# Luoyadan/CRB-active-3Ddet

Hardware: AMD Instinct MI355X
Metric: frames/s SECOND fwd+bwd, KITTI 20k-pt clouds (higher is better)
Workload: dtype f32

## Files before the change

crb-active-3ddet_amd/crbhip/bnrelu.py:

```python
import torch

from ._lib import lib, check, ptr, cur_stream, require_cuda


FUSE_RUNNING = __import__('os').environ.get('CRB_BN_FUSE_RUNNING', '1') == '1'
TICKETS = __import__('os').environ.get('CRB_BN_TICKETS', '1') == '1'
_ticket_areas = {}


def _scratch(dev, wsb):
    ws = torch.empty((wsb,), dtype=torch.uint8, device=dev)
    if not TICKETS:
        return ws, None
    key = (dev.index, torch.cuda.current_stream(dev).cuda_stream)
    t = _ticket_areas.get(key)
    if t is None:
        t = _ticket_areas[key] = torch.zeros((lib.crb_bn_ticket_ints(),), dtype=torch.int32, device=dev)
    return ws, t


def _bn_check(rc, what):
    if rc != 0:
        _ticket_areas.clear()
    check(rc, what)
# ... 260 lines not shown
            zptr = ctypes.c_void_p(out.data_ptr() + 4 * col)
            _bn_check(lib.crb_bn_relu_forward(ptr(x), n, C, ptr(g), ptr(b), float(eps), int(relu), zptr, total, ptr(mean),
                                          ptr(var), ptr(invstd), ptr(rm), ptr(rv), None, float(mom), ptr(ws), wsb, ptr(tk),
                                          cur_stream(dev)), 'crb_bn_relu_forward')
            _touch(rm, rv)
            saved += [x, mean, invstd, g, b]
            col += C
        ctx.save_for_backward(*saved)
        ctx.relu, ctx.widths = int(relu), widths
        return out

    @staticmethod
    def backward(ctx, dz):
        import ctypes
        dz = dz.contiguous().float()
        n, total = dz.shape
        saved = ctx.saved_tensors
        grads, col = [None], 0
        for i, C in enumerate(ctx.widths):
            x, mean, invstd, g, b = saved[5 * i:5 * i + 5]
            dev = x.device
            dx = torch.empty_like(x)
            dgamma = torch.empty((C,), dtype=torch.float32, device=dev)
            dbeta = torch.empty_like(dgamma)
            wsb = lib.crb_bn_workspace_bytes(n, C)
            ws, tk = _scratch(dev, wsb)
            dzp = ctypes.c_void_p(dz.data_ptr() + 4 * col)
            _bn_check(lib.crb_bn_relu_backward(ptr(x), dzp, total, n, C, ptr(mean), ptr(invstd), ptr(g), ptr(b), ctx.relu,
                                           ptr(dx), ptr(dgamma), ptr(dbeta), ptr(ws), wsb, ptr(tk), cur_stream(dev)),
                  'crb_bn_relu_backward')
            grads += [dx, dgamma, dbeta, None, None, None, None]
            col += C
        return tuple(grads)


def bn_relu_concat(xs, bns, relu=True):
    if _GROUPS is not None and _GROUPS.G > 1:
        off = _GROUPS.offsets(xs[0])
        if not torch.is_grad_enabled():
            total = sum(x.shape[1] for x in xs)
            out = torch.empty((xs[0].shape[0], total), dtype=torch.float32, device=xs[0].device)
            col = 0
            for x, bn in zip(xs, bns):
                _frames_forward(x, off, bn, relu, out, col)
                col += x.shape[1]
            return out
        with frame_groups(1):
            return torch.cat([bn_relu_concat([x[a:b] for x in xs], bns, relu) for a, b in zip(off[:-1], off[1:])], 0)
    args = []
    for x, bn in zip(xs, bns):
        with torch.no_grad():
            bn.num_batches_tracked += 1
        args += [x, bn.weight, bn.bias, bn.eps, bn.running_mean, bn.running_var, float(bn.momentum)]
    return _BNReLUConcatTrain.apply(relu, *args)


class _BNReLUMaxConcatTrain(torch.autograd.Function):

    @staticmethod
    def forward(ctx, *args):
        import ctypes
        k = len(args) // 8
        xs = [args[8 * i].contiguous() for i in range(k)]
        nss = [int(args[8 * i + 1]) for i in range(k)]
        dev = xs[0].device
        M = xs[0].shape[0] // nss[0]
        widths = [x.shape[1] for x in xs]
        total = sum(widths)
        out = torch.empty((M, total), dtype=torch.float32, device=dev)
        saved, col = [], 0
        for i, x in enumerate(xs):
            gamma, beta, eps, rm, rv, mom = args[8 * i + 2:8 * i + 8]
            C, ns = widths[i], nss[i]
            assert x.shape[0] == M * ns
            mean = torch.empty((C,), dtype=torch.float32, device=dev)
            var, invstd = torch.empty_like(mean), torch.empty_like(mean)
            arg = torch.empty((M, C), dtype=torch.int32, device=dev)
            wsb = lib.crb_bn_workspace_bytes(M * ns, C)
            ws, tk = _scratch(dev, wsb)
            g, b = gamma.contiguous().float(), beta.contiguous().float()
            zptr = ctypes.c_void_p(out.data_ptr() + 4 * col)
            _bn_check(lib.crb_bn_relu_max_forward(ptr(x), M, ns, C, ptr(g), ptr(b), float(eps), zptr, total, ptr(arg),
                                              ptr(mean), ptr(var), ptr(invstd), ptr(rm), ptr(rv), None, float(mom), ptr(ws), wsb,
                                              ptr(tk), cur_stream(dev)), 'crb_bn_relu_max_forward')
            _touch(rm, rv)
            saved += [x, mean, invstd, g, b, arg]
            col += C
        ctx.save_for_backward(*saved)
        ctx.widths, ctx.nss = widths, nss
        return out

    @staticmethod
    def backward(ctx, gz):
        import ctypes
        gz = gz.contiguous().float()
        M, total = gz.shape
        saved = ctx.saved_tensors
        grads, col = [], 0
        for i, (C, ns) in enumerate(zip(ctx.widths, ctx.nss)):
            x, mean, invstd, g, b, arg = saved[6 * i:6 * i + 6]
            dev = x.device
            dx = torch.empty_like(x)
            dgamma = torch.empty((C,), dtype=torch.float32, device=dev)
            dbeta = torch.empty_like(dgamma)
            wsb = lib.crb_bn_workspace_bytes(M * ns, C)
            ws, tk = _scratch(dev, wsb)
            gp = ctypes.c_void_p(gz.data_ptr() + 4 * col)
# ... 46 lines not shown
```

crb-active-3ddet_amd/csrc/bn_relu.hip:

```cpp
#include "crb_common.h"
#include "../../include/crb_hip.h"

typedef float f4 __attribute__((ext_vector_type(4)));

namespace {

static inline int bn_rows_per_block(int64_t n) {
  int64_t r = (n + 1023) / 1024;
  r = r < 128 ? 128 : r;
  return (int)r;
}

CRB_KNOB g_bn_order = 2;

constexpr int BN_GROUPS = 32;
struct BnFinal {
  int* tickets;
  double* group;
  float* o0;
  float* o1;
  float* o2;
  float* running_mean;
  float* running_var;
  long long* num_batches_tracked;
  float momentum, eps;
  int64_t n;
  int bwd;
};

__device__ __forceinline__ void st_agent(float* p, float v) {
  __hip_atomic_store(p, v, __ATOMIC_RELAXED, __HIP_MEMORY_SCOPE_AGENT);
}
__device__ __forceinline__ void st_agent4(float* p, f4 v) {
  st_agent(p, v[0]);
  st_agent(p + 1, v[1]);
  st_agent(p + 2, v[2]);
  st_agent(p + 3, v[3]);
}

__device__ __forceinline__ void bn_ticket_finalize(const float* partial, int nblk, int C, int blk, const BnFinal& f) {
  __shared__ int s_role;
  asm volatile("s_waitcnt vmcnt(0)" ::: "memory");
  __syncthreads();
  const int ngroups = nblk < BN_GROUPS ? nblk : BN_GROUPS;
  const int grp = blk % BN_GROUPS;
  const int members = (nblk - grp + BN_GROUPS - 1) / BN_GROUPS;
  if (threadIdx.x == 0)
    s_role = __hip_atomic_fetch_add(&f.tickets[1 + grp], 1, __ATOMIC_RELAXED, __HIP_MEMORY_SCOPE_AGENT) == members - 1 ? 1 : 0;
  __syncthreads();
  if (!s_role) return;
  const int C2 = 2 * C;
  for (int i = threadIdx.x; i < C2; i += 256) {
    double a = 0.0;
    int k = grp;
    for (; k + 7 * BN_GROUPS < nblk; k += 8 * BN_GROUPS) {
      float v[8];
// ... 387 lines not shown
                                                              const float* __restrict__ gamma, const float* __restrict__ beta,
                                                              float* __restrict__ z, int C, int relu, int64_t ld_z,
                                                              BnFrames fr) {
  const int f = blockIdx.y;
  const int64_t rows = fr.off[f + 1] - fr.off[f];
  const int64_t t = (int64_t)blockIdx.x * 256 + threadIdx.x;
  if (t * 4 >= rows * C) return;
  const int c = (int)((t * 4) % C);
  const int64_t row = fr.off[f] + (t * 4) / C;
  const float* st = stats + (int64_t)f * 4 * C;
  const f4 v = *reinterpret_cast<const f4*>(x + row * C + c);
  const f4 mu = *reinterpret_cast<const f4*>(st + c), is = *reinterpret_cast<const f4*>(st + 2 * C + c);
  const f4 ga = *reinterpret_cast<const f4*>(gamma + c), be = *reinterpret_cast<const f4*>(beta + c);
  f4 o = ga * ((v - mu) * is) + be;
  if (relu) {
#pragma unroll
    for (int k = 0; k < 4; ++k) o[k] = o[k] > 0.f ? o[k] : 0.f;
  }
  *reinterpret_cast<f4*>(z + row * ld_z + c) = o;
}

__global__ __launch_bounds__(256) void bn_relu_max_frames_kernel(const float* __restrict__ x, const float* __restrict__ stats,
                                                                 const float* __restrict__ gamma, const float* __restrict__ beta,
                                                                 int64_t groups, int64_t groups_per_frame, int ns, int C,
                                                                 float* __restrict__ zmax, int64_t ld_out,
                                                                 int* __restrict__ arg) {
  const int c4n = C >> 2;
  const int tc = threadIdx.x % c4n, tr = threadIdx.x / c4n;
  const int glanes = 256 / c4n;
  if (tr >= glanes) return;
  const int64_t m = (int64_t)blockIdx.x * glanes + tr;
  if (m >= groups) return;
  const int c = tc * 4;
  const float* st = stats + (m / groups_per_frame) * 4 * C;
  const f4 mu = *reinterpret_cast<const f4*>(st + c), is = *reinterpret_cast<const f4*>(st + 2 * C + c);
  const f4 ga = *reinterpret_cast<const f4*>(gamma + c), be = *reinterpret_cast<const f4*>(beta + c);
  const float* src = x + m * ns * C + c;
  f4 best = (f4){-1.f, -1.f, -1.f, -1.f};
  int bi[4] = {0, 0, 0, 0};
  for (int s = 0; s < ns; ++s) {
    const f4 v = *reinterpret_cast<const f4*>(src + (int64_t)s * C);
    f4 o = ga * ((v - mu) * is) + be;
#pragma unroll
    for (int k = 0; k < 4; ++k) {
      o[k] = o[k] > 0.f ? o[k] : 0.f;
      if (o[k] > best[k]) { best[k] = o[k]; bi[k] = s; }
    }
  }
  *reinterpret_cast<f4*>(zmax + m * ld_out + c) = best;
  int* a = arg + m * C + c;
  a[0] = bi[0]; a[1] = bi[1]; a[2] = bi[2]; a[3] = bi[3];
}

}

static inline int bn_blocks(int64_t n) { return crb_cdiv(n, bn_rows_per_block(n)); }

static inline int64_t bn_partial_bytes(int64_t n, int C) { return crb_align_up((int64_t)bn_blocks(n) * 2 * C * 4, 256); }
extern "C" int64_t crb_bn_workspace_bytes(int64_t n, int C) {
  return bn_partial_bytes(n, C) + (int64_t)BN_GROUPS * 2 * C * 8 + 256;
}
extern "C" int crb_bn_ticket_ints(void) { return 1 + BN_GROUPS; }

static inline BnFinal bn_final(int32_t* tickets, void* workspace, int64_t n, int C, int bwd, float* o0, float* o1, float* o2,
                               float* running_mean, float* running_var, float momentum, float eps,
                               int64_t* num_batches_tracked = nullptr) {
  BnFinal f;
  f.tickets = tickets;
  f.group = reinterpret_cast<double*>(static_cast<char*>(workspace) + bn_partial_bytes(n, C));
  f.o0 = o0;
  f.o1 = o1;
  f.o2 = o2;
  f.running_mean = running_mean;
  f.running_var = running_var;
  f.num_batches_tracked = reinterpret_cast<long long*>(num_batches_tracked);
  f.momentum = momentum;
  f.eps = eps;
  f.n = n;
  f.bwd = bwd;
  return f;
}

extern "C" int crb_bn_relu_forward(const float* x, int64_t n, int C, const float* gamma, const float* beta, float eps,
                                   int relu, float* z, int64_t z_row_stride, float* mean, float* var, float* invstd,
                                   float* running_mean, float* running_var, int64_t* num_batches_tracked, float momentum,
                                   void* workspace, int64_t workspace_bytes, int32_t* tickets, void* stream) {
  const int64_t ld_z = z_row_stride > 0 ? z_row_stride : C;
  if (ld_z < C || (ld_z & 3)) return CRB_ERR_ARG;
  if (n <= 0 || C <= 0 || (C & 3) || C > 1024 || (256 % (C >> 2) && (C >> 2) < 256)) return CRB_ERR_ARG;
  if (workspace_bytes < crb_bn_workspace_bytes(n, C) - 256 || !workspace) return CRB_ERR_WORKSPACE;
  hipStream_t st = (hipStream_t)stream;
  const int nblk = bn_blocks(n);
  float* partial = (float*)workspace;
  hipLaunchKernelGGL(bn_partial_kernel<false>, dim3(nblk), dim3(256), 2 * 256 * 16, st, x, nullptr, nullptr, nullptr,
                     nullptr, nullptr, n, C, relu, bn_rows_per_block(n), (int64_t)C, partial, g_bn_order & 1,
                     bn_final(tickets, workspace, n, C, 0, mean, var, invstd, running_mean, running_var, momentum, eps,
                              num_batches_tracked));
  if (!tickets)
    hipLaunchKernelGGL(bn_finalize_kernel, dim3(crb_cdiv(C, 8)), dim3(256), 0, st, partial, nblk, C, n, eps, 0, mean, var,
                       invstd, running_mean, running_var, momentum, reinterpret_cast<long long*>(num_batches_tracked));
  const int64_t total4 = n * C / 4;
  if (z)
    hipLaunchKernelGGL(bn_apply_kernel, dim3(crb_cdiv(total4, 256)), dim3(256), 0, st, x, mean, invstd, gamma, beta, z,
                       total4, C, relu, ld_z, (g_bn_order >> 1) & 1);
  CRB_CHECK_LAUNCH();
  return CRB_OK;
// ... 25 lines not shown
  if (workspace_bytes < crb_bn_workspace_bytes(n, C) - 256 || !workspace) return CRB_ERR_WORKSPACE;
  hipStream_t st = (hipStream_t)stream;
  const int nblk = (int)(n_slabs < bn_blocks(n) ? n_slabs : bn_blocks(n));
  float* partial = (float*)workspace;
  hipLaunchKernelGGL(bn_slab_partial_kernel, dim3(nblk), dim3(256), 0, st, slab_sums, n_slabs, C, partial,
                     bn_final(tickets, workspace, n, C, 0, mean, var, invstd, running_mean, running_var, momentum, eps,
                              num_batches_tracked));
  if (!tickets)
    hipLaunchKernelGGL(bn_finalize_kernel, dim3(crb_cdiv(C, 8)), dim3(256), 0, st, partial, nblk, C, n, eps, 0, mean, var,
                       invstd, running_mean, running_var, momentum, reinterpret_cast<long long*>(num_batches_tracked));
  const int64_t total4 = n * C / 4;
  if (z)
    hipLaunchKernelGGL(bn_apply_kernel, dim3(crb_cdiv(total4, 256)), dim3(256), 0, st, x, mean, invstd, gamma, beta, z,
                       total4, C, relu, ld_z, (g_bn_order >> 1) & 1);
  CRB_CHECK_LAUNCH();
  return CRB_OK;
}

extern "C" int crb_bn_relu_apply(const float* x, int64_t n, int C, const float* mean, const float* invstd,
                                 const float* gamma, const float* beta, int relu, float* z, int64_t z_row_stride,
                                 void* stream) {
  if (n < 0 || C <= 0 || (C & 3)) return CRB_ERR_ARG;
  const int64_t ld_z = z_row_stride > 0 ? z_row_stride : C;
  if (ld_z < C || (ld_z & 3)) return CRB_ERR_ARG;
  if (n == 0) return CRB_OK;
  const int64_t total4 = n * C / 4;
  hipLaunchKernelGGL(bn_apply_kernel, dim3(crb_cdiv(total4, 256)), dim3(256), 0, (hipStream_t)stream, x, mean, invstd,
                     gamma, beta, z, total4, C, relu, ld_z, 0);
  CRB_CHECK_LAUNCH();
  return CRB_OK;
}

extern "C" int crb_bn_relu_backward(const float* x, const float* dz, int64_t dz_row_stride, int64_t n, int C, const float* mean,
                                    const float* invstd, const float* gamma, const float* beta, int relu, float* dx,
                                    float* dgamma, float* dbeta, void* workspace, int64_t workspace_bytes, int32_t* tickets,
                                    void* stream) {
  if (n <= 0 || C <= 0 || (C & 3) || C > 1024 || (256 % (C >> 2) && (C >> 2) < 256)) return CRB_ERR_ARG;
  if (workspace_bytes < crb_bn_workspace_bytes(n, C) - 256 || !workspace) return CRB_ERR_WORKSPACE;
  const int64_t ld_dz = dz_row_stride > 0 ? dz_row_stride : C;
  if (ld_dz < C || (ld_dz & 3)) return CRB_ERR_ARG;
  hipStream_t st = (hipStream_t)stream;
  const int nblk = bn_blocks(n);
  float* partial = (float*)workspace;
  hipLaunchKernelGGL(bn_partial_kernel<true>, dim3(nblk), dim3(256), 2 * 256 * 16, st, x, dz, mean, invstd, gamma, beta, n,
                     C, relu, bn_rows_per_block(n), ld_dz, partial, g_bn_order & 1,
                     bn_final(tickets, workspace, n, C, 1, dbeta, dgamma, nullptr, nullptr, nullptr, 0.f, 0.f));
  if (!tickets)
    hipLaunchKernelGGL(bn_finalize_kernel, dim3(crb_cdiv(C, 8)), dim3(256), 0, st, partial, nblk, C, n, 0.f, 1, dbeta, dgamma,
                       (float*)nullptr, (float*)nullptr, (float*)nullptr, 0.f);
  const int64_t total4 = n * C / 4;
  if (dx)
    hipLaunchKernelGGL(bn_bwd_apply_kernel, dim3(crb_cdiv(total4, 256)), dim3(256), 0, st, x, dz, mean, invstd, gamma, beta,
                       dbeta, dgamma, dx, total4, C, 1.0f / (float)n, relu, ld_dz, (g_bn_order >> 1) & 1);
  CRB_CHECK_LAUNCH();
  return CRB_OK;
}

#ifdef CRB_MEASURE
extern "C" int crb_bn_relu_backward_partials(const float* x, const float* dz, int64_t dz_row_stride, int64_t n, int C,
                                             const float* slab_sums, int64_t n_slabs, const float* mean, const float* invstd,
                                             const float* gamma, const float* beta, int relu, float* dx, float* dgamma, float* dbeta,
                                             void* workspace, int64_t workspace_bytes, int32_t* tickets, void* stream) {
  if (n <= 0 || C <= 0 || (C & 3) || C > 1024 || (256 % (C >> 2) && (C >> 2) < 256) || !slab_sums || n_slabs <= 0) return CRB_ERR_ARG;
  if (workspace_bytes < crb_bn_workspace_bytes(n, C) - 256 || !workspace) return CRB_ERR_WORKSPACE;
  const int64_t ld_dz = dz_row_stride > 0 ? dz_row_stride : C;
  if (ld_dz < C || (ld_dz & 3)) return CRB_ERR_ARG;
  hipStream_t st = (hipStream_t)stream;
  const int nblk = (int)(n_slabs < bn_blocks(n) ? n_slabs : bn_blocks(n));
  float* partial = (float*)workspace;
  hipLaunchKernelGGL(bn_slab_partial_kernel, dim3(nblk), dim3(256), 0, st, slab_sums, n_slabs, C, partial,
                     bn_final(tickets, workspace, n, C, 1, dbeta, dgamma, nullptr, nullptr, nullptr, 0.f, 0.f));
  if (!tickets)
    hipLaunchKernelGGL(bn_finalize_kernel, dim3(crb_cdiv(C, 8)), dim3(256), 0, st, partial, nblk, C, n, 0.f, 1, dbeta, dgamma,
                       (float*)nullptr, (float*)nullptr, (float*)nullptr, 0.f);
  const int64_t total4 = n * C / 4;
  if (dx)
    hipLaunchKernelGGL(bn_bwd_apply_kernel, dim3(crb_cdiv(total4, 256)), dim3(256), 0, st, x, dz, mean, invstd, gamma, beta,
                       dbeta, dgamma, dx, total4, C, 1.0f / (float)n, relu, ld_dz, (g_bn_order >> 1) & 1);
  CRB_CHECK_LAUNCH();
  return CRB_OK;
}
#endif

extern "C" int crb_bn_relu_max_forward(const float* x, int64_t groups, int ns, int C, const float* gamma, const float* beta,
                                       float eps, float* zmax, int64_t out_row_stride, int32_t* arg, float* mean, float* var,
                                       float* invstd, float* running_mean, float* running_var,
                                       int64_t* num_batches_tracked, float momentum, void* workspace,
                                       int64_t workspace_bytes, int32_t* tickets, void* stream) {
  const int64_t n = groups * ns;
  const int64_t ld = out_row_stride > 0 ? out_row_stride : C;
  if (ld < C || (ld & 3) || ns <= 0) return CRB_ERR_ARG;
  if (n <= 0 || C <= 0 || (C & 3) || C > 1024 || (256 % (C >> 2) && (C >> 2) < 256)) return CRB_ERR_ARG;
  if (workspace_bytes < crb_bn_workspace_bytes(n, C) - 256 || !workspace) return CRB_ERR_WORKSPACE;
  hipStream_t st = (hipStream_t)stream;
  const int nblk = bn_blocks(n);
  float* partial = (float*)workspace;
  hipLaunchKernelGGL(bn_partial_kernel<false>, dim3(nblk), dim3(256), 2 * 256 * 16, st, x, nullptr, nullptr, nullptr,
                     nullptr, nullptr, n, C, 1, bn_rows_per_block(n), (int64_t)C, partial, 0,
                     bn_final(tickets, workspace, n, C, 0, mean, var, invstd, running_mean, running_var, momentum, eps,
                              num_batches_tracked));
  if (!tickets)
    hipLaunchKernelGGL(bn_finalize_kernel, dim3(crb_cdiv(C, 8)), dim3(256), 0, st, partial, nblk, C, n, eps, 0, mean, var,
                       invstd, running_mean, running_var, momentum, reinterpret_cast<long long*>(num_batches_tracked));
  const int glanes = 256 / (C >> 2) > 0 ? 256 / (C >> 2) : 1;
  hipLaunchKernelGGL(bn_relu_max_kernel, dim3(crb_cdiv(groups, glanes)), dim3(256), 0, st, x, mean, invstd, gamma, beta,
                     groups, ns, C, zmax, ld, arg);
// ... 172 lines not shown
```

crb-active-3ddet_amd/pcdet/models/backbones_2d/base_bev_backbone.py:

```python
import numpy as np
import torch
import torch.nn as nn

from crbhip import bnrelu

from ...utils.fold_utils import fold_conv_bn
from ...utils.linear_rows import LinearRows, rows_view, rows_to_nchw


ROWS_TRAIN = True
ROWS_GEMM = True
WINOGRAD = __import__('os').environ.get('CRB_WINOGRAD', '1') != '0'


def _wino_fold(w, shift):
    from crbhip import winograd
    return winograd.weights_forward2(w), shift.contiguous()


def _wino_ok(conv, x, pad=None):
    if not WINOGRAD or not isinstance(conv, nn.Conv2d) or not x.is_cuda or x.dtype != torch.float32:
        return False
    from crbhip import winograd
    p = tuple(conv.padding) if pad is None else tuple(pad)
# ... 189 lines not shown
    def forward(self, data_dict):
        spatial_features = data_dict['spatial_features']
        ups = []
        x = spatial_features
        if not self.training and not torch.is_grad_enabled():
            cat_ok = x.is_cuda and x.is_contiguous(memory_format=torch.channels_last) and self._can_fuse_concat_eval(x)
            pre = []
            for i, blk in enumerate(self.blocks):
                x = self._run_folded(blk, x)
                if cat_ok:
                    pre.append(self._up(self.deblocks[i][0], x))
                else:
                    ups.append(self._run_folded(self.deblocks[i], x) if len(self.deblocks) > 0 else x)
            if cat_ok and all(p.is_contiguous(memory_format=torch.channels_last) and p.shape[2:] == pre[0].shape[2:]
                              for p in pre):
                n, _, h, w_ = pre[0].shape
                cat = torch.empty((n * h * w_, sum(p.shape[1] for p in pre)), dtype=torch.float32, device=x.device)
                col = 0
                for d, p in zip(self.deblocks, pre):
                    bnrelu.bn_apply_into(p.permute(0, 2, 3, 1).reshape(n * h * w_, p.shape[1]), d[1], True, cat, col)
                    col += p.shape[1]
                ups = [cat.view(n, h, w_, cat.shape[1]).permute(0, 3, 1, 2)]
            elif cat_ok:
                ups = [self._run_folded(nn.Sequential(*list(d)[1:]), p) for d, p in zip(self.deblocks, pre)]
            x = torch.cat(ups, dim=1) if len(ups) > 1 else ups[0]
            if len(self.deblocks) > len(self.blocks):
                x = self._run_folded(self.deblocks[-1], x)
            data_dict['spatial_features_2d'] = x
            return data_dict
        run = self._run_rows_train if (ROWS_TRAIN and x.is_cuda and x.is_contiguous(memory_format=torch.channels_last)) \
            else (lambda seq, t: seq(t))
        if run == self._run_rows_train and torch.is_grad_enabled():
            from crbhip import winograd
            if winograd.PREPARE:
                winograd.prepare_weights2([m.weight for blk in self.blocks for m in blk
                                           if isinstance(m, nn.Conv2d) and m.kernel_size == (3, 3) and m.stride == (1, 1)
                                           and m.weight.is_cuda])
        fuse_cat = ROWS_TRAIN and x.is_cuda and self._can_fuse_concat(x)
        pre = []
        for i, blk in enumerate(self.blocks):
            x = run(blk, x)
            stride = int(spatial_features.shape[2] / x.shape[2])
            data_dict['spatial_features_%dx' % stride] = x
            if fuse_cat:
                pre.append(self._up(self.deblocks[i][0], x))
            else:
                ups.append(run(self.deblocks[i], x) if len(self.deblocks) > 0 else x)
        if fuse_cat and all(p.is_contiguous(memory_format=torch.channels_last) and p.shape[2:] == pre[0].shape[2:]
                            for p in pre):
            n, _, h, w_ = pre[0].shape
            rows = [p.permute(0, 2, 3, 1).reshape(n * h * w_, p.shape[1]) for p in pre]
            cat = bnrelu.bn_relu_concat(rows, [d[1] for d in self.deblocks[:len(pre)]], relu=True)
            ups = [cat.view(n, h, w_, cat.shape[1]).permute(0, 3, 1, 2)]
        elif fuse_cat:
            ups = [d[2](d[1](p)) for d, p in zip(self.deblocks, pre)]
        x = torch.cat(ups, dim=1) if len(ups) > 1 else ups[0]
        if len(self.deblocks) > len(self.blocks):
            x = self.deblocks[-1](x)
        data_dict['spatial_features_2d'] = x
        if x.is_cuda:
            from crbhip import winograd
            winograd.forget_prepared_forward()
        return data_dict
```

crb-active-3ddet_amd/pcdet/models/dense_heads/anchor_head_single.py:

```python
import numpy as np
import torch
import torch.nn as nn

from ...utils.linear_rows import LinearRows, rows_view
from .anchor_head_template import AnchorHeadTemplate


FUSED_HEAD_CONVS = True
ROWS_GEMM = True


class AnchorHeadSingle(AnchorHeadTemplate):
    def __init__(self, model_cfg, input_channels, num_class, class_names, grid_size, point_cloud_range,
                 predict_boxes_when_training=True, **kwargs):
        super().__init__(model_cfg=model_cfg, num_class=num_class, class_names=class_names, grid_size=grid_size,
                         point_cloud_range=point_cloud_range, predict_boxes_when_training=predict_boxes_when_training)
        self.num_anchors_per_location = sum(self.num_anchors_per_location)
        n = self.num_anchors_per_location
        self.conv_cls = nn.Conv2d(input_channels, n * self.num_class, kernel_size=1)
        self.conv_box = nn.Conv2d(input_channels, n * self.box_coder.code_size, kernel_size=1)
        if self.model_cfg.get('USE_DIRECTION_CLASSIFIER', None) is not None:
            self.conv_dir_cls = nn.Conv2d(input_channels, n * self.model_cfg.NUM_DIR_BINS, kernel_size=1)
        else:
            self.conv_dir_cls = None
        self.lazy_box_decode = False
        self.init_weights()

    def init_weights(self):
        pi = 0.01
        nn.init.constant_(self.conv_cls.bias, -np.log((1 - pi) / pi))
        nn.init.normal_(self.conv_box.weight, mean=0, std=0.001)

    def forward(self, data_dict):
        feats = data_dict['spatial_features_2d']
        if FUSED_HEAD_CONVS:
            heads = [self.conv_cls, self.conv_box] + ([self.conv_dir_cls] if self.conv_dir_cls is not None else [])
            w = torch.cat([h.weight for h in heads], 0)
            b = torch.cat([h.bias for h in heads], 0)
            rows = rows_view(feats) if (ROWS_GEMM and feats.is_cuda) else None
            if rows is not None:
                n, _, h, w_ = feats.shape
                y = LinearRows.apply(rows, w.flatten(1), b).view(n, h, w_, w.shape[0])
            else:
                y = torch.nn.functional.conv2d(feats, w, b).permute(0, 2, 3, 1)
            outs = torch.split(y, [h.out_channels for h in heads], dim=3)
            cls_preds, box_preds = outs[0].contiguous(), outs[1].contiguous()
            dir_cls_preds = outs[2].contiguous() if self.conv_dir_cls is not None else None
        else:
            cls_preds = self.conv_cls(feats).permute(0, 2, 3, 1).contiguous()
            box_preds = self.conv_box(feats).permute(0, 2, 3, 1).contiguous()
            dir_cls_preds = None
            if self.conv_dir_cls is not None:
                dir_cls_preds = self.conv_dir_cls(feats).permute(0, 2, 3, 1).contiguous()
        self.forward_ret_dict['cls_preds'] = cls_preds
        self.forward_ret_dict['box_preds'] = box_preds
        self.forward_ret_dict['dir_cls_preds'] = dir_cls_preds
        if self.training:
            self.forward_ret_dict.update(self.assign_targets(gt_boxes=data_dict['gt_boxes']))
        if not self.training or self.predict_boxes_when_training:
            B = data_dict['batch_size']
            data_dict['rpn_preds'] = cls_preds
            data_dict['cls_preds_normalized'] = False
            if self.lazy_box_decode:
                data_dict['batch_cls_preds'] = cls_preds.view(B, -1, self.num_class).float()
                data_dict['batch_box_decoder'] = lambda idx: self.generate_predicted_boxes(
                    batch_size=B, cls_preds=cls_preds, box_preds=box_preds, dir_cls_preds=dir_cls_preds, anchor_idx=idx)[1]
                data_dict.pop('batch_box_preds', None)
            else:
                batch_cls_preds, batch_box_preds = self.generate_predicted_boxes(
                    batch_size=B, cls_preds=cls_preds, box_preds=box_preds, dir_cls_preds=dir_cls_preds)
                data_dict['batch_cls_preds'] = batch_cls_preds
                data_dict['batch_box_preds'] = batch_box_preds
        return data_dict
```

include/crb_hip.h:

```cpp
#ifndef CRB_HIP_H
#define CRB_HIP_H
#include <stdint.h>

#ifdef __cplusplus
extern "C" {
#endif

#define CRB_OK 0
#define CRB_ERR_ARG (-1)
#define CRB_ERR_WORKSPACE (-2)
#define CRB_ERR_LAUNCH (-3)
#define CRB_ERR_UNSUPPORTED (-4)

int crb_abi_version(void);

int64_t crb_voxelize_workspace_bytes(int64_t n_points, int B, int max_voxels, int max_points);
int crb_voxelize(const float* points, int64_t n_points, int num_features,
                 const int32_t* frame_offsets, int B,
                 const float* range_min_xyz, const float* voxel_size_xyz, const int32_t* grid_xyz,
                 int max_voxels, int max_points,
                 float* voxels, int32_t* coords, int32_t* num_points, float* mean_features,
                 int32_t* num_voxels_out,
                 void* workspace, int64_t workspace_bytes, void* stream);

// ... 223 lines not shown
int64_t crb_pair_sort_workspace_bytes(int64_t M, int nsample);
int crb_pair_sort_by_source(int B, int64_t M, int nsample, const int32_t* xyz_batch_cnt, const int32_t* new_xyz_batch_cnt,
                            const int32_t* idx, const uint8_t* empty_mask, int64_t n_src, int32_t* sorted_pair,
                            int32_t* sorted_row, void* workspace, int64_t workspace_bytes, void* stream);
int crb_sorted_key_counts(const void* key, int key_is_float, int64_t stride, int64_t n, int B, int32_t* counts, void* stream);
int crb_voxel_centers(const int32_t* coords_zyx, int64_t row_stride, int64_t n, const float* scaled_voxel_size, const float* range_min,
                      float* out, void* stream);
int crb_farthest_point_sample(int B, int n, int m, const float* xyz, float* temp, int32_t* out_idx, void* stream);
int crb_three_nn_stack(int B, int64_t N, const float* unknown, const int32_t* unknown_batch_cnt,
                       const float* known, const int32_t* known_batch_cnt, float* dist2, int32_t* idx,
                       void* stream);
int crb_three_interpolate_stack(int64_t N, int C, const float* features, const int32_t* idx,
                                const float* weight, float* out, void* stream);
int crb_three_interpolate_grad_stack(int64_t N, int C, const float* grad_out, const int32_t* idx,
                                     const float* weight, float* grad_features, void* stream);

int crb_points_in_boxes(int B, int T, int M, const float* boxes, const float* pts, int32_t* box_idx_of_points,
                        void* stream);
int64_t crb_gt_point_stats_workspace_bytes(int B, int G, int C);
int crb_gt_point_stats(int B, int G, int C, int64_t N, int stride, const float* pts, const int32_t* frame_offsets,
                       const float* gt_boxes, float* stats, void* workspace, int64_t workspace_bytes, void* stream);
int crb_roiaware_pool3d_forward(int N, int P, int C, int max_pts_each_voxel, int out_x, int out_y, int out_z,
                                const float* rois, const float* pts, const float* pts_feature,
                                int32_t* argmax, int32_t* pts_idx_of_voxels, float* pooled_features,
                                int pool_method, void* stream);
int crb_roiaware_pool3d_backward(int N, int C, int max_pts_each_voxel, int out_x, int out_y, int out_z,
                                 const int32_t* pts_idx_of_voxels, const int32_t* argmax,
                                 const float* grad_out, float* grad_in, int pool_method, void* stream);

int64_t crb_density_greedy_workspace_bytes(int n_candidates, int num_class);
int crb_density_greedy(const float* densities, const int32_t* labels, int n_candidates, int dmax,
                       int num_class, const double* xaxis, const double* prior, double bandwidth,
                       int select_nums, int32_t* order, double* best_scores, void* workspace,
                       int64_t workspace_bytes, void* stream);

int64_t crb_bn_workspace_bytes(int64_t n, int C);
int crb_bn_ticket_ints(void);
int crb_bn_relu_forward(const float* x, int64_t n, int C, const float* gamma, const float* beta, float eps,
                        int relu, float* z, int64_t z_row_stride, float* mean, float* var, float* invstd,
                        float* running_mean, float* running_var, int64_t* num_batches_tracked, float momentum,
                        void* workspace, int64_t workspace_bytes, int32_t* tickets, void* stream);
int crb_bn_relu_forward_partials(const float* x, int64_t n, int C, const float* slab_sums, int64_t n_slabs, const float* gamma,
                                 const float* beta, float eps, int relu, float* z, int64_t z_row_stride, float* mean, float* var,
                                 float* invstd, float* running_mean, float* running_var, int64_t* num_batches_tracked,
                                 float momentum, void* workspace, int64_t workspace_bytes, int32_t* tickets, void* stream);
int crb_bn_affine_table(const float* mean, const float* invstd, const float* gamma, const float* beta, int C, float* out_c2,
                        void* stream);
int crb_bn_relu_apply(const float* x, int64_t n, int C, const float* mean, const float* invstd,
                      const float* gamma, const float* beta, int relu, float* z, int64_t z_row_stride, void* stream);
int crb_bn_relu_backward(const float* x, const float* dz, int64_t dz_row_stride, int64_t n, int C, const float* mean,
                         const float* invstd, const float* gamma, const float* beta, int relu, float* dx,
                         float* dgamma, float* dbeta, void* workspace, int64_t workspace_bytes, int32_t* tickets,
                         void* stream);
int crb_bn_relu_max_forward(const float* x, int64_t groups, int ns, int C, const float* gamma, const float* beta, float eps,
                            float* zmax, int64_t out_row_stride, int32_t* arg, float* mean, float* var, float* invstd,
                            float* running_mean, float* running_var, int64_t* num_batches_tracked, float momentum,
                            void* workspace, int64_t workspace_bytes, int32_t* tickets, void* stream);
int crb_bn_relu_max_backward(const float* x, const float* gz, int64_t gz_row_stride, const int32_t* arg, int64_t groups,
                             int ns, int C, const float* mean, const float* invstd, const float* gamma, const float* beta,
                             float* dx, float* dgamma, float* dbeta, void* workspace, int64_t workspace_bytes,
                             int32_t* tickets, void* stream);
int crb_bn_relu_max_backward_sums(const float* x_sel, const float* gz, int64_t gz_row_stride, int64_t groups, int C,
                                  const float* mean, const float* invstd, const float* gamma, const float* beta, float* dgamma,
                                  float* dbeta, void* workspace, int64_t workspace_bytes, int32_t* tickets, void* stream);
int64_t crb_bn_frames_workspace_bytes(int n_frames, int64_t max_rows_per_frame, int C);
int crb_bn_relu_forward_frames(const float* x, int n_frames, const int64_t* frame_row_offsets, int C, const float* gamma,
                               const float* beta, float eps, int relu, float* z, int64_t z_row_stride,
                               float* running_mean, float* running_var, float momentum, void* workspace,
                               int64_t workspace_bytes, void* stream);
int crb_bn_relu_max_forward_frames(const float* x, int n_frames, int64_t groups_per_frame, int ns, int C,
                                   const float* gamma, const float* beta, float eps, float* zmax, int64_t out_row_stride,
                                   int32_t* arg, float* running_mean, float* running_var, float momentum, void* workspace,
                                   int64_t workspace_bytes, void* stream);

int64_t crb_assign_targets_workspace_bytes(int B, int A, int G);
int crb_assign_targets(const float* anchors, const int32_t* anchor_cls, int A, const float* gt_boxes,
                       const uint8_t* gt_valid, int B, int G, const float* matched_thr,
                       const float* unmatched_thr, int32_t* labels, float* reg_targets, float* reg_weights,
                       void* workspace, int64_t workspace_bytes, void* stream);

typedef struct CrbRpnLossCfg {
  float alpha, gamma;
  float beta;
  float dir_offset;
  float code_weights[7];
  float cls_weight, loc_weight, dir_weight;
  int32_t num_class, num_dir_bins;
} CrbRpnLossCfg;
int64_t crb_rpn_loss_workspace_bytes(int B, int A);
int crb_rpn_loss_forward(const float* cls_preds, const float* box_preds, const float* dir_preds, const int32_t* labels,
                         const float* reg_targets, const float* anchors, int B, int A, const CrbRpnLossCfg* cfg,
                         float* loss, float* npos, void* workspace, int64_t workspace_bytes, void* stream);
int crb_rpn_loss_backward(const float* cls_preds, const float* box_preds, const float* dir_preds, const int32_t* labels,
                          const float* reg_targets, const float* anchors, int B, int A, const CrbRpnLossCfg* cfg,
                          const float* npos, const float* grad_loss, float* d_cls, float* d_box, float* d_dir, void* stream);

int crb_decode_selected_anchors(const float* box_preds, const float* dir_preds, const float* anchors, const int64_t* anchor_idx, int B,
                                int64_t A, int k, int num_dir_bins, float dir_offset, float dir_limit_offset, float* out, void* stream);
int crb_proposal_finish(const int32_t* keep, const int64_t* top_idx, const float* top_boxes, const float* scores, const int64_t* labels,
                        const float* cls_preds, int B, int64_t A, int k, int post, int box_row_stride, int num_class, float* rois,
                        float* roi_scores, int64_t* roi_labels, float* full_cls_scores, void* stream);

int crb_point_labels(const int32_t* inner, const int32_t* outer, const float* gt_boxes, int B, int64_t M, int G, int gt_row_stride,
                     int num_class, int64_t* labels, void* stream);
int crb_point_focal_loss(const float* preds, const int64_t* labels, int64_t n, int num_class, float alpha, float gamma,
                         float loss_weight, float* loss, float* d_preds, void* stream);
// ... 217 lines not shown
```

Measured before the change: 480.2.

## Fuse detection-head GEMM backward into BN-ReLU-concat backward via low-rank MFMA kernels

Adds a fused autograd path for the BEV concat feeding the 1x1 head conv. The head's input gradient (dy·W) is recomputed on the fly per 16-row tile with MFMA inside the BN-ReLU backward partial and apply kernels, so the wide concat gradient never has to be materialised. The aim is to avoid writing and reading back the full n×C_total activation gradient. In exchange the small GEMM is computed twice (once in the partial pass, once in the apply pass), and the path depends on tensor data_ptr matching, supported channel widths, and K ≤ 72.

```diff
diff --git a/crb-active-3ddet_amd/crbhip/bnrelu.py b/crb-active-3ddet_amd/crbhip/bnrelu.py
--- a/crb-active-3ddet_amd/crbhip/bnrelu.py
+++ b/crb-active-3ddet_amd/crbhip/bnrelu.py
@@ -336,7 +336,81 @@
         with torch.no_grad():
             bn.num_batches_tracked += 1
         args += [x, bn.weight, bn.bias, bn.eps, bn.running_mean, bn.running_var, float(bn.momentum)]
-    return _BNReLUConcatTrain.apply(relu, *args)
+    out = _BNReLUConcatTrain.apply(relu, *args)
+    if CONCAT_HEAD and out.grad_fn is not None:
+        out._crb_concat_head = ConcatHandle(out, xs, bns, out.grad_fn.saved_tensors, relu)
+    return out
+
+
+CONCAT_HEAD = __import__('os').environ.get('CRB_CONCAT_HEAD', '1') == '1'
+
+
+class ConcatHandle(object):
+
+    def __init__(self, cat, xs, bns, saved, relu):
+        self.key = (cat.data_ptr(), tuple(cat.shape))
+        self.xs, self.bns, self.saved, self.relu = list(xs), list(bns), tuple(saved), int(relu)
+        self.widths = [int(x.shape[1]) for x in xs]
+
+    def matches(self, rows):
+        return rows.data_ptr() == self.key[0] and tuple(rows.shape) == self.key[1] and rows.is_contiguous()
+
+
+def concat_head_supported(handle, rows, K):
+    return (CONCAT_HEAD and handle is not None and torch.is_grad_enabled() and handle.matches(rows) and
+            all(lib.crb_bn_relu_backward_lowrank_supported(C, int(K)) == 1 for C in handle.widths))
+
+
+class _ConcatHead(torch.autograd.Function):
+
+    @staticmethod
+    def forward(ctx, cat, w, b, handle, *leaves):
+        ctx.save_for_backward(cat, w, *handle.saved)
+        ctx.relu, ctx.widths = handle.relu, handle.widths
+        return torch.addmm(b, cat, w.t())
+
+    @staticmethod
+    def backward(ctx, dy):
+        import ctypes
+        from pcdet.utils.linear_rows import tall_t_matmul
+        saved = ctx.saved_tensors
+        cat, w = saved[0], saved[1]
+        dy = dy.contiguous().float()
+        n, K = dy.shape
+        total = w.shape[1]
+        w = w.contiguous()
+        dw = tall_t_matmul(dy, cat) if ctx.needs_input_grad[1] else None
+        db = dy.sum(0) if ctx.needs_input_grad[2] else None
+        grads, col = [None, dw, db, None], 0
+        for i, C in enumerate(ctx.widths):
+            x, mean, invstd, g, be = saved[2 + 5 * i:7 + 5 * i]
+            need = ctx.needs_input_grad[4 + 3 * i:7 + 3 * i]
+            if not any(need):
+                grads += [None, None, None]
+                col += C
+                continue
+            dev = x.device
+            dx = torch.empty_like(x) if need[0] else None
+            dgamma = torch.empty((C,), dtype=torch.float32, device=dev)
+            dbeta = torch.empty_like(dgamma)
+            wsb = lib.crb_bn_workspace_bytes(n, C)
+            ws, tk = _scratch(dev, wsb)
+            e0 = _prof_begin()
+            _bn_check(lib.crb_bn_relu_backward_lowrank(ptr(x), n, C, ptr(dy), K, K, ctypes.c_void_p(w.data_ptr() + 4 * col), total,
+                                                       ptr(mean), ptr(invstd), ptr(g), ptr(be), ctx.relu, ptr(dx), ptr(dgamma),
+                                                       ptr(dbeta), ptr(ws), wsb, ptr(tk), cur_stream(dev)),
+                      'crb_bn_relu_backward_lowrank')
+            _prof_end(e0, 'bn_bwd_lowrank', n, C)
+            grads += [dx, dgamma if need[1] else None, dbeta if need[2] else None]
+            col += C
+        return tuple(grads)
+
+
+def concat_head(cat_rows, handle, w, b):
+    leaves = []
+    for x, bn in zip(handle.xs, handle.bns):
+        leaves += [x, bn.weight, bn.bias]
+    return _ConcatHead.apply(cat_rows.detach(), w, b, handle, *leaves)
 
 
 class _BNReLUMaxConcatTrain(torch.autograd.Function):
diff --git a/crb-active-3ddet_amd/csrc/bn_relu.hip b/crb-active-3ddet_amd/csrc/bn_relu.hip
--- a/crb-active-3ddet_amd/csrc/bn_relu.hip
+++ b/crb-active-3ddet_amd/csrc/bn_relu.hip
@@ -2,6 +2,7 @@
 #include "../../include/crb_hip.h"
 
 typedef float f4 __attribute__((ext_vector_type(4)));
+typedef double d4 __attribute__((ext_vector_type(4)));
 
 namespace {
 
@@ -495,6 +496,219 @@
   a[0] = bi[0]; a[1] = bi[1]; a[2] = bi[2]; a[3] = bi[3];
 }
 
+constexpr int LR_TPW = 4;
+constexpr int LR_CW = 16 * LR_TPW;
+constexpr int LR_KMAX = 72;
+constexpr int LR_CHAINS = 3;
+constexpr int LR_LDZ = LR_CW + 4;
+constexpr int LR_STAGE = 16 * LR_KMAX + 16 * LR_LDZ;
+
+__device__ __forceinline__ void lr_wave_sync() {
+  __builtin_amdgcn_fence(__ATOMIC_RELEASE, "wavefront");
+  __builtin_amdgcn_wave_barrier();
+  __builtin_amdgcn_fence(__ATOMIC_ACQUIRE, "wavefront");
+}
+
+template <int KS, bool EXACT>
+struct LrWave {
+  float wf[LR_TPW][KS];
+  float nd[KS];
+  float* sdy;
+  float* sdz;
+  int lane, K;
+
+  __device__ __forceinline__ void init(float* stage, const float* __restrict__ w, int64_t ld_w, int K_, int cbase) {
+    lane = threadIdx.x & 63;
+    K = EXACT ? 4 * KS : K_;
+    sdy = stage;
+    sdz = stage + 16 * LR_KMAX;
+    const int j = lane & 15, g = lane >> 4;
+#pragma unroll
+    for (int t = 0; t < LR_TPW; ++t)
+#pragma unroll
+      for (int s = 0; s < KS; ++s) {
+        const int k = 4 * s + g;
+        wf[t][s] = k < K ? w[(int64_t)k * ld_w + cbase + 16 * t + j] : 0.f;
+      }
+  }
+  __device__ __forceinline__ void fetch_dy(const float* __restrict__ dy, int64_t row0, int64_t r1) {
+    const float* p = dy + row0 * K + lane;
+    if (EXACT && row0 + 16 <= r1) {
+#pragma unroll
+      for (int i = 0; i < KS; ++i) nd[i] = p[64 * i];
+    } else {
+      const int64_t left = r1 - row0;
+      const int lim = (left < 0 ? 0 : (left > 16 ? 16 : (int)left)) * K;
+#pragma unroll
+      for (int i = 0; i < KS; ++i) nd[i] = lane + 64 * i < lim ? p[64 * i] : 0.f;
+    }
+  }
+  __device__ __forceinline__ void stage_dy() {
+#pragma unroll
+    for (int i = 0; i < KS; ++i)
+      if (EXACT || lane + 64 * i < 16 * K) sdy[lane + 64 * i] = nd[i];
+    lr_wave_sync();
+  }
+  __device__ __forceinline__ void products(f4 (&d)[4]) {
+    const int j = lane & 15, g = lane >> 4;
+    float bf[KS];
+#pragma unroll
+    for (int s = 0; s < KS; ++s) bf[s] = (EXACT || 4 * s + g < K) ? sdy[j * K + 4 * s + g] : 0.f;
+    f4 acc[LR_CHAINS][LR_TPW];
+#pragma unroll
+    for (int h = 0; h < LR_CHAINS; ++h)
+#pragma unroll
+      for (int t = 0; t < LR_TPW; ++t) acc[h][t] = (f4){0, 0, 0, 0};
+#pragma unroll
+    for (int s = 0; s < KS; ++s)
+#pragma unroll
+      for (int t = 0; t < LR_TPW; ++t)
+        acc[s % LR_CHAINS][t] = __builtin_amdgcn_mfma_f32_16x16x4f32(wf[t][s], bf[s], acc[s % LR_CHAINS][t], 0, 0, 0);
+#pragma unroll
+    for (int t = 0; t < LR_TPW; ++t) {
+      f4 v = acc[0][t];
+#pragma unroll
+      for (int h = 1; h < LR_CHAINS; ++h) v += acc[h][t];
+      *reinterpret_cast<f4*>(sdz + j * LR_LDZ + 16 * t + 4 * g) = v;
+    }
+    lr_wave_sync();
+#pragma unroll
+    for (int i = 0; i < 4; ++i) d[i] = *reinterpret_cast<const f4*>(sdz + (g + 4 * i) * LR_LDZ + 4 * j);
+    lr_wave_sync();
+  }
+};
+
+__device__ __forceinline__ void lr_load_x(f4 (&xv)[4], const float* __restrict__ x, int64_t row, int64_t r1, int C, int c, bool full) {
+  const float* p = x + row * C + c;
+  if (full) {
+#pragma unroll
+    for (int i = 0; i < 4; ++i) xv[i] = *reinterpret_cast<const f4*>(p + (int64_t)(4 * i) * C);
+  } else {
+#pragma unroll
+    for (int i = 0; i < 4; ++i)
+      xv[i] = row + 4 * i < r1 ? *reinterpret_cast<const f4*>(p + (int64_t)(4 * i) * C) : (f4){0, 0, 0, 0};
+  }
+}
+
+__device__ __forceinline__ void lr_after(f4 (&xv)[4], const f4 (&d)[4]) {
+#pragma unroll
+  for (int i = 0; i < 4; ++i) asm volatile("" : "+v"(xv[i]) : "v"(d[i]));
+}
+
+template <int KS, bool EXACT>
+__global__ __launch_bounds__(256, 2) void bn_lr_partial_kernel(const float* __restrict__ x, const float* __restrict__ dy,
+                                                               int K, const float* __restrict__ w, int64_t ld_w,
+                                                               const float* __restrict__ mean, const float* __restrict__ invstd,
+                                                               const float* __restrict__ gamma, const float* __restrict__ beta,
+                                                               int64_t n, int C, int relu, int rows_per_block,
+                                                               float* __restrict__ partial, int reversed, BnFinal fin) {
+  __shared__ __attribute__((aligned(32))) float smem[4 * LR_STAGE];
+  const int wave = threadIdx.x >> 6;
+  const int CG = C / LR_CW, RG = 4 / CG;
+  const int cbase = (wave % CG) * LR_CW, rg = wave / CG;
+  const int blk = reversed ? gridDim.x - 1 - blockIdx.x : blockIdx.x;
+  const int64_t r0 = (int64_t)blk * rows_per_block;
+  const int64_t r1 = min(n, r0 + rows_per_block);
+  LrWave<KS, EXACT> lw;
+  lw.init(smem + wave * LR_STAGE, w, ld_w, K, cbase);
+  const int cq = lw.lane & 15, rq = lw.lane >> 4;
+  const int c = cbase + 4 * cq;
+  const f4 mu = *reinterpret_cast<const f4*>(mean + c), is = *reinterpret_cast<const f4*>(invstd + c);
+  const f4 ga = *reinterpret_cast<const f4*>(gamma + c), be = *reinterpret_cast<const f4*>(beta + c);
+  d4 a = (d4){0, 0, 0, 0}, b = (d4){0, 0, 0, 0};
+  const int ntile = (int)((r1 - r0 + 15) >> 4);
+  lw.fetch_dy(dy, r0 + rg * 16, r1);
+  for (int tile = rg; tile < ntile; tile += RG) {
+    const int64_t row0 = r0 + tile * 16;
+    const bool full = row0 + 16 <= r1;
+    lw.stage_dy();
+    f4 xv[4];
+    lr_load_x(xv, x, row0 + rq, r1, C, c, full);
+    lw.fetch_dy(dy, row0 + RG * 16, r1);
+    f4 d[4];
+    lw.products(d);
+    lr_after(xv, d);
+#pragma unroll
+    for (int i = 0; i < 4; ++i) {
+      const f4 xh = (xv[i] - mu) * is;
+      f4 dd = d[i];
+      if (relu) {
+        const f4 z = ga * xh + be;
+#pragma unroll
+        for (int k = 0; k < 4; ++k) dd[k] = z[k] > 0.f ? dd[k] : 0.f;
+      }
+      if (!full && row0 + rq + 4 * i >= r1) dd = (f4){0, 0, 0, 0};
+      a += __builtin_convertvector(dd, d4);
+      b += __builtin_convertvector(dd * xh, d4);
+    }
+  }
+  __syncthreads();
+  const int RL = 4 * RG, ldr = C + 8;
+  double* red = reinterpret_cast<double*>(smem);
+  *reinterpret_cast<d4*>(red + (0 * RL + rg * 4 + rq) * ldr + c) = a;
+  *reinterpret_cast<d4*>(red + (1 * RL + rg * 4 + rq) * ldr + c) = b;
+  __syncthreads();
+  for (int i = threadIdx.x; i < 2 * C; i += 256) {
+    const int which = i / C, ch = i - which * C;
+    double acc = 0.0;
+    for (int rl = 0; rl < RL; ++rl) acc += red[(which * RL + rl) * ldr + ch];
+    const float v = (float)acc;
+    if (fin.tickets) st_agent(partial + (int64_t)blk * 2 * C + i, v);
+    else partial[(int64_t)blk * 2 * C + i] = v;
+  }
+  if (fin.tickets) bn_ticket_finalize(partial, gridDim.x, C, blk, fin);
+}
+
+template <int KS, bool EXACT>
+__global__ __launch_bounds__(256, 2) void bn_lr_apply_kernel(const float* __restrict__ x, const float* __restrict__ dy,
+                                                             int K, const float* __restrict__ w, int64_t ld_w,
+                                                             const float* __restrict__ mean, const float* __restrict__ invstd,
+                                                             const float* __restrict__ gamma, const float* __restrict__ beta,
+                                                             const float* __restrict__ dbeta, const float* __restrict__ dgamma,
+                                                             float* __restrict__ dx, int64_t n, int C, float inv_n, int relu,
+                                                             int rows_per_block, int reversed) {
+  __shared__ __attribute__((aligned(16))) float smem[4 * LR_STAGE];
+  const int wave = threadIdx.x >> 6;
+  const int CG = C / LR_CW, RG = 4 / CG;
+  const int cbase = (wave % CG) * LR_CW, rg = wave / CG;
+  const int blk = reversed ? gridDim.x - 1 - blockIdx.x : blockIdx.x;
+  const int64_t r0 = (int64_t)blk * rows_per_block;
+  const int64_t r1 = min(n, r0 + rows_per_block);
+  LrWave<KS, EXACT> lw;
+  lw.init(smem + wave * LR_STAGE, w, ld_w, K, cbase);
+  const int cq = lw.lane & 15, rq = lw.lane >> 4;
+  const int c = cbase + 4 * cq;
+  const f4 mu = *reinterpret_cast<const f4*>(mean + c), is = *reinterpret_cast<const f4*>(invstd + c);
+  const f4 ga = *reinterpret_cast<const f4*>(gamma + c), be = *reinterpret_cast<const f4*>(beta + c);
+  const f4 db = *reinterpret_cast<const f4*>(dbeta + c), dg = *reinterpret_cast<const f4*>(dgamma + c);
+  const int ntile = (int)((r1 - r0 + 15) >> 4);
+  lw.fetch_dy(dy, r0 + rg * 16, r1);
+  for (int tile = rg; tile < ntile; tile += RG) {
+    const int64_t row0 = r0 + tile * 16;
+    const bool full = row0 + 16 <= r1;
+    lw.stage_dy();
+    f4 xv[4];
+    lr_load_x(xv, x, row0 + rq, r1, C, c, full);
+    lw.fetch_dy(dy, row0 + RG * 16, r1);
+    f4 d[4];
+    lw.products(d);
+    lr_after(xv, d);
+    float* q = dx + (row0 + rq) * C + c;
+#pragma unroll
+    for (int i = 0; i < 4; ++i) {
+      const f4 xh = (xv[i] - mu) * is;
+      f4 dd = d[i];
+      if (relu) {
+        const f4 z = ga * xh + be;
+#pragma unroll
+        for (int k = 0; k < 4; ++k) dd[k] = z[k] > 0.f ? dd[k] : 0.f;
+      }
+      if (full || row0 + rq + 4 * i < r1)
+        *reinterpret_cast<f4*>(q + (int64_t)(4 * i) * C) = ga * is * (dd - db * inv_n - xh * (dg * inv_n));
+    }
+  }
+}
+
 }
 
 static inline int bn_blocks(int64_t n) { return crb_cdiv(n, bn_rows_per_block(n)); }
@@ -626,6 +840,52 @@
   if (dx)
     hipLaunchKernelGGL(bn_bwd_apply_kernel, dim3(crb_cdiv(total4, 256)), dim3(256), 0, st, x, dz, mean, invstd, gamma, beta,
                        dbeta, dgamma, dx, total4, C, 1.0f / (float)n, relu, ld_dz, (g_bn_order >> 1) & 1);
+  CRB_CHECK_LAUNCH();
+  return CRB_OK;
+}
+
+extern "C" int crb_bn_relu_backward_lowrank_supported(int C, int K) {
+  return (C == 64 || C == 128 || C == 256) && K >= 1 && K <= 72;
+}
+
+template <int KS, bool EXACT>
+static void bn_lr_launch(const float* x, int64_t n, int C, const float* dy, int K, const float* w, int64_t ld_w,
+                         const float* mean, const float* invstd, const float* gamma, const float* beta, int relu, float* dx,
+                         float* dgamma, float* dbeta, void* workspace, int32_t* tickets, hipStream_t st) {
+  const int nblk = bn_blocks(n), rpb = bn_rows_per_block(n);
+  float* partial = (float*)workspace;
+  hipLaunchKernelGGL((bn_lr_partial_kernel<KS, EXACT>), dim3(nblk), dim3(256), 0, st, x, dy, K, w, ld_w, mean, invstd, gamma, beta,
+                     n, C, relu, rpb, partial, g_bn_order & 1,
+                     bn_final(tickets, workspace, n, C, 1, dbeta, dgamma, nullptr, nullptr, nullptr, 0.f, 0.f));
+  if (!tickets)
+    hipLaunchKernelGGL(bn_finalize_kernel, dim3(crb_cdiv(C, 8)), dim3(256), 0, st, partial, nblk, C, n, 0.f, 1, dbeta, dgamma,
+                       (float*)nullptr, (float*)nullptr, (float*)nullptr, 0.f);
+  if (dx)
+    hipLaunchKernelGGL((bn_lr_apply_kernel<KS, EXACT>), dim3(nblk), dim3(256), 0, st, x, dy, K, w, ld_w, mean, invstd, gamma, beta,
+                       dbeta, dgamma, dx, n, C, 1.0f / (float)n, relu, rpb, (g_bn_order >> 1) & 1);
+}
+
+extern "C" int crb_bn_relu_backward_lowrank(const float* x, int64_t n, int C, const float* dy, int64_t dy_row_stride, int K,
+                                            const float* w, int64_t w_row_stride, const float* mean, const float* invstd,
+                                            const float* gamma, const float* beta, int relu, float* dx, float* dgamma,
+                                            float* dbeta, void* workspace, int64_t workspace_bytes, int32_t* tickets,
+                                            void* stream) {
+  if (n <= 0 || !crb_bn_relu_backward_lowrank_supported(C, K)) return CRB_ERR_ARG;
+  const int64_t ld_w = w_row_stride > 0 ? w_row_stride : C;
+  if ((dy_row_stride != 0 && dy_row_stride != K) || ld_w < C) return CRB_ERR_ARG;
+  if (!x || !dy || !w || !mean || !invstd || !gamma || !beta || !dgamma || !dbeta) return CRB_ERR_ARG;
+  if (((uintptr_t)x & 15) || ((uintptr_t)dx & 15)) return CRB_ERR_ARG;
+  if (workspace_bytes < crb_bn_workspace_bytes(n, C) - 256 || !workspace) return CRB_ERR_WORKSPACE;
+  hipStream_t st = (hipStream_t)stream;
+#define LR_GO(KS, EXACT)                                                                                                  \
+  bn_lr_launch<KS, EXACT>(x, n, C, dy, K, w, ld_w, mean, invstd, gamma, beta, relu, dx, dgamma, dbeta, workspace, tickets, st)
+  if (K == 20) LR_GO(5, true);
+  else if (K < 20) LR_GO(5, false);
+  else if (K == 40) LR_GO(10, true);
+  else if (K < 40) LR_GO(10, false);
+  else if (K == 72) LR_GO(18, true);
+  else LR_GO(18, false);
+#undef LR_GO
   CRB_CHECK_LAUNCH();
   return CRB_OK;
 }
diff --git a/crb-active-3ddet_amd/pcdet/models/backbones_2d/base_bev_backbone.py b/crb-active-3ddet_amd/pcdet/models/backbones_2d/base_bev_backbone.py
--- a/crb-active-3ddet_amd/pcdet/models/backbones_2d/base_bev_backbone.py
+++ b/crb-active-3ddet_amd/pcdet/models/backbones_2d/base_bev_backbone.py
@@ -265,6 +265,7 @@
             rows = [p.permute(0, 2, 3, 1).reshape(n * h * w_, p.shape[1]) for p in pre]
             cat = bnrelu.bn_relu_concat(rows, [d[1] for d in self.deblocks[:len(pre)]], relu=True)
             ups = [cat.view(n, h, w_, cat.shape[1]).permute(0, 3, 1, 2)]
+            ups[0]._crb_concat_head = getattr(cat, '_crb_concat_head', None)
         elif fuse_cat:
             ups = [d[2](d[1](p)) for d, p in zip(self.deblocks, pre)]
         x = torch.cat(ups, dim=1) if len(ups) > 1 else ups[0]
diff --git a/crb-active-3ddet_amd/pcdet/models/dense_heads/anchor_head_single.py b/crb-active-3ddet_amd/pcdet/models/dense_heads/anchor_head_single.py
--- a/crb-active-3ddet_amd/pcdet/models/dense_heads/anchor_head_single.py
+++ b/crb-active-3ddet_amd/pcdet/models/dense_heads/anchor_head_single.py
@@ -1,6 +1,8 @@
 import numpy as np
 import torch
 import torch.nn as nn
+
+from crbhip import bnrelu
 
 from ...utils.linear_rows import LinearRows, rows_view
 from .anchor_head_template import AnchorHeadTemplate
@@ -40,7 +42,11 @@
             rows = rows_view(feats) if (ROWS_GEMM and feats.is_cuda) else None
             if rows is not None:
                 n, _, h, w_ = feats.shape
-                y = LinearRows.apply(rows, w.flatten(1), b).view(n, h, w_, w.shape[0])
+                handle = getattr(feats, '_crb_concat_head', None)
+                if bnrelu.concat_head_supported(handle, rows, w.shape[0]):
+                    y = bnrelu.concat_head(rows, handle, w.flatten(1), b).view(n, h, w_, w.shape[0])
+                else:
+                    y = LinearRows.apply(rows, w.flatten(1), b).view(n, h, w_, w.shape[0])
             else:
                 y = torch.nn.functional.conv2d(feats, w, b).permute(0, 2, 3, 1)
             outs = torch.split(y, [h.out_channels for h in heads], dim=3)
diff --git a/include/crb_hip.h b/include/crb_hip.h
--- a/include/crb_hip.h
+++ b/include/crb_hip.h
@@ -299,6 +299,11 @@
                          const float* invstd, const float* gamma, const float* beta, int relu, float* dx,
                          float* dgamma, float* dbeta, void* workspace, int64_t workspace_bytes, int32_t* tickets,
                          void* stream);
+int crb_bn_relu_backward_lowrank_supported(int C, int K);
+int crb_bn_relu_backward_lowrank(const float* x, int64_t n, int C, const float* dy, int64_t dy_row_stride, int K, const float* w,
+                                 int64_t w_row_stride, const float* mean, const float* invstd, const float* gamma,
+                                 const float* beta, int relu, float* dx, float* dgamma, float* dbeta, void* workspace,
+                                 int64_t workspace_bytes, int32_t* tickets, void* stream);
 int crb_bn_relu_max_forward(const float* x, int64_t groups, int ns, int C, const float* gamma, const float* beta, float eps,
                             float* zmax, int64_t out_row_stride, int32_t* arg, float* mean, float* var, float* invstd,
                             float* running_mean, float* running_var, int64_t* num_batches_tracked, float momentum,
```

Result: no change. 483.2, median of 6 (+0.6%).
